# hieucnm/GNN-RecSys

Hardware: AMD Instinct MI355X
Metric: edges aggregated/sec, full-graph embed pass, d=128 (higher is better)
Workload: dtype fp32

## Files before the change

gnn-recsys_amd/csrc/pack_rows.hpp:

```cpp
#pragma once
#include <cstdint>
#include <cstring>

namespace gnnrec {

constexpr int kPackD = 128;
constexpr int kPackWords = 96;
constexpr int kPackHdrWords = 8;
constexpr int kPackSlots = kPackWords - kPackHdrWords;
constexpr uint32_t kPackDenseBit = 0x80000000u;
constexpr int kPackStatusWords = 4;
constexpr double kPackMaxDenseFrac = 1.0 / 8;

inline void pack_row_host(const float* x, uint32_t* p) {
  uint32_t bits[kPackD];
  std::memcpy(bits, x, sizeof(bits));
  for (int i = 0; i < kPackWords; ++i) p[i] = 0;
  uint32_t nnz = 0, pre = 0;
  for (int w = 0; w < 4; ++w) {
    pre |= nnz << (8 * w);
    for (int b = 0; b < 32; ++b)
      if (bits[32 * w + b] != 0) {
        p[w] |= 1u << b;
        ++nnz;
      }
  }
  p[4] = pre;
// ... 21 lines not shown
```

gnn-recsys_amd/csrc/rowq.hpp:

```cpp
#pragma once
#include <hip/hip_runtime.h>
#include <cstdint>

namespace gnnrec {

constexpr int kRqHeads = 8;
constexpr int kRqStride = 32;
constexpr int kRqSlotWords = (kRqHeads + 1) * kRqStride;

unsigned* rowq_slot(hipStream_t stream, int* ticket);
void rowq_launched(int ticket, hipStream_t stream);
constexpr int kScanMaxTiles = 4096;
constexpr int kScanFlags0 = 16;
constexpr int kScanSlotWords = kScanFlags0 + kScanMaxTiles;
constexpr unsigned kScanSlots = 128;
unsigned long long* scan_slot(hipStream_t stream, int* ticket);
void scan_launched(int ticket, hipStream_t stream);
int device_cus();
int cu_reserve();

inline int64_t persistent_blocks(int64_t units, int per_cu) {
  const int64_t cus = device_cus() - cu_reserve();
  const int64_t blocks = per_cu * (cus > 8 ? cus : 8);
  return units < blocks ? units : blocks;
}

inline unsigned* rowq_slot_for(int64_t n_dst, int64_t drawers, int rq_ch, hipStream_t stream,
                               int* ticket) {
  return n_dst >= drawers * rq_ch * 4 ? rowq_slot(stream, ticket) : nullptr;
}

__device__ inline int xcc_id() {
  return __builtin_amdgcn_s_getreg((3 << 11) | 20) & (kRqHeads - 1);
}

__device__ inline unsigned rq_take(unsigned* head) {
  unsigned t = 0;
// ... 138 lines not shown
```

gnn-recsys_amd/csrc/spmm.hip:

```cpp
#include "common.hpp"
#include "dropout.hpp"
#include "gather.hpp"
#include "rowq.hpp"
#include <cmath>
#include <cstdlib>
#include <type_traits>

namespace gnnrec {
namespace {

constexpr int64_t kRqTicketEdges = 512;
constexpr int64_t kRqMinRowsPerWave = 32;
constexpr int kRowChunk = 0;
constexpr int64_t kGroupMaxAvgDeg = 16;

__device__ __forceinline__ int ticket_rows(int64_t avg_deg, int64_t n_dst, int64_t waves) {
  int64_t c = kRqTicketEdges / (avg_deg > 0 ? avg_deg : 1);
  const int64_t cap = n_dst / (waves * 4);
  if (c > cap) c = cap;
  return (int)(c < 1 ? 1 : c > 64 ? 64 : c);
}

struct HeavyPlan {
  int64_t split;
// ... 416 lines not shown
  int where;
};

struct SpmmArgs {
  const char* name;
  const int64_t* indptr; const int32_t* indices; const float* ew; const float* X; int64_t ldx;
  int64_t n_dst; float* out; int64_t ldo; int flags;
  HeavyPlan hp;
  float* ws;
  const int64_t* live;
  const uint32_t* P;
  const int* pstatus;
  const DropCall* drop;
  int d;
  DropArgs da;
};

SpmmArgs spmm_args(const char* name, const int64_t* indptr, const int32_t* indices,
                   const float* ew, const float* X, int64_t ldx, int64_t n_dst, float* out,
                   int64_t ldo, int flags) {
  SpmmArgs a{};
  a.name = name;
  a.indptr = indptr; a.indices = indices; a.ew = ew; a.X = X; a.ldx = ldx;
  a.n_dst = n_dst; a.out = out; a.ldo = ldo; a.flags = flags;
  return a;
}

constexpr int64_t kBlocksPerCu = 8;

inline unsigned grid_waves(int64_t units) {
  int64_t blocks = (units + 3) / 4;
  const int cus = device_cus() - cu_reserve();
  const int64_t max_blocks = (int64_t)(cus > 8 ? cus : 8) * kBlocksPerCu;
  if (blocks > max_blocks) blocks = max_blocks;
  return (unsigned)(blocks < 1 ? 1 : blocks);
}

template <class P, class C>
int launch_family(const SpmmArgs& a, hipStream_t s, const P& p, const C& c, const char* what) {
  const int cols_per_slice = P::LPR * P::VEC;
  const unsigned slices = (unsigned)((a.d + cols_per_slice - 1) / cols_per_slice);
  const int64_t max_deg = a.hp.n_heavy > 0 ? a.hp.split : INT64_MAX;
  const unsigned grid = grid_waves(a.n_dst);
  const int flags = a.flags & (GNNREC_SPMM_EMPTY_NEGINF | GNNREC_SPMM_ACCUM);
  int ticket = -1;
  unsigned* rq = nullptr;
  if constexpr (P::kQueue)
    if (slices == 1 && a.n_dst >= (int64_t)grid * 4 * kRqMinRowsPerWave) rq = rowq_slot(s, &ticket);
  hipLaunchKernelGGL((spmm_csr_kernel<P>), dim3(grid, slices), dim3(256), 0, s, a.indptr,
                     a.indices, a.n_dst, a.d, a.out, a.ldo, flags, max_deg, rq, kRowChunk,
                     kGroupMaxAvgDeg, P::kLive ? a.live : nullptr, a.hp.counts, p);
  if constexpr (P::kQueue) rowq_launched(ticket, s);
  if (a.hp.n_heavy > 0) {
    hipLaunchKernelGGL((spmm_chunk_kernel<C>), dim3(grid_waves(a.hp.n_chunks), slices), dim3(256),
                       0, s, a.indptr, a.indices, a.d, a.hp, a.ws, c);
    const unsigned cslices = (unsigned)((a.d + 64 * P::VEC - 1) / (64 * P::VEC));
    hipLaunchKernelGGL((spmm_combine_kernel<typename P::Finish>),
                       dim3(grid_waves(a.hp.n_heavy), cslices), dim3(256), 0, s, a.indptr, a.d,
// ... 116 lines not shown
    a.da = DropArgs{a.drop->keys, (int)a.drop->key_index, dp.T, dp.scale, (int)((d + 3) / 4)};
  }
  const bool vec4 = (d % 4 == 0) && (a.ldx % 4 == 0) && (a.ldo % 4 == 0) && aligned16(a.X) &&
                    aligned16(a.out) && (a.hp.n_heavy == 0 || aligned16(a.ws));
  int lpr = 64;
  if (vec4) {
    const int64_t lanes = d / 4;
    lpr = 4;
    while (lpr < lanes && lpr < 64) lpr <<= 1;
  }
  hipStream_t s = as_stream(stream);
  return vec4 ? dispatch_reduce<4>(reduce, lpr, a, s) : dispatch_reduce<1>(reduce, lpr, a, s);
}

}
}

extern "C" int gnnrec_spmm_csr_f32(const int64_t* indptr, const int32_t* indices, const float* ew,
                                   const float* X, int64_t ldx, int64_t n_dst, int64_t d,
                                   int reduce, int flags, float* out, int64_t ldo, void* stream) {
  return gnnrec_spmm_csr_live_f32(indptr, indices, ew, X, ldx, n_dst, d, reduce, flags, out, ldo,
                                  nullptr, stream);
}

extern "C" int gnnrec_spmm_csr_packed_f32(const int64_t* indptr, const int32_t* indices,
                                          const void* packed, const int32_t* status,
                                          const float* X, int64_t ldx, int64_t n_dst, int64_t d,
                                          int reduce, int flags, float* out, int64_t ldo,
                                          int64_t split, const int64_t* heavy_rows,
                                          int64_t n_heavy, const int64_t* chunk_ptr,
// ... 365 lines not shown
```

gnn-recsys_amd/csrc/spmm_project.hip:

```cpp
#include "common.hpp"
#include "gather.hpp"
#include "rowq.hpp"
#include <cstdlib>
#include <type_traits>

namespace gnnrec {
namespace {

constexpr int kPD = 128;
constexpr int kPWaves = 16;
constexpr int kPRows = 2;
constexpr int kFusedChunk = 8;

struct EpiArgs {
  bool relu, l2, attn;
  int accum;
  float out_div, a0, a1;
  float* attn_state;
  float* out;
  int64_t ldo;
  int j0;
};

__device__ __forceinline__ void epilogue_row(const EpiArgs& e, int64_t row, bool valid,
// ... 415 lines not shown
  }
  if (rq != nullptr) rq_finish(rq);
}

}
}

using namespace gnnrec;

static int launch_spmm_project(const char* name, const int64_t* indptr, const int32_t* indices,
                               const float* ew, const float* X, int64_t ldx, const float* H,
                               int64_t ldh, const float* W_selfT, const float* W_neighT,
                               const float* bias, const float* bias_nonempty, int64_t n_dst,
                               int64_t d, int reduce, int epilogue, int accum, float out_div,
                               const float* attn_vec, float* attn_state, float* out, int64_t ldo,
                               float* agg, int64_t lda, int agg_mode, void* stream) {
  GNNREC_REQUIRE(reduce == GNNREC_REDUCE_SUM || reduce == GNNREC_REDUCE_MEAN ||
                     reduce == GNNREC_REDUCE_MAX,
                 "%s: unknown reduce %d", name, reduce);
  GNNREC_REQUIRE(agg_mode == GNNREC_AGG_NONE || agg_mode == GNNREC_AGG_SAVE ||
                     agg_mode == GNNREC_AGG_LOAD,
                 "%s: unknown aggregate mode %d", name, agg_mode);
  const bool load = agg_mode == GNNREC_AGG_LOAD;
  const int st = load ? fused_check(name, d, epilogue, false, accum, attn_vec, attn_state, n_dst,
                                    'X', {indptr, H, W_selfT}, {H, W_selfT, W_neighT}, {ldh}, out,
                                    ldo)
                      : fused_check(name, d, epilogue, false, accum, attn_vec, attn_state, n_dst,
                                    'X', {indptr, X, H, W_selfT}, {X, H, W_selfT, W_neighT},
                                    {ldx, ldh}, out, ldo);
  if (st != GNNREC_OK || n_dst == 0) return st;
  GNNREC_REQUIRE(W_neighT, "%s: W_neighT = NULL (pre-projected source "
                           "rows) is gnnrec_spmm_project_mfma_f32's form", name);
  if (agg_mode != GNNREC_AGG_NONE) {
    GNNREC_REQUIRE(agg, "%s: the aggregate mode needs agg", name);
    GNNREC_REQUIRE(aligned16(agg) && lda >= kPD && lda % 4 == 0,
                   "%s: agg needs 16-B aligned rows of lda >= %d floats", name, kPD);
  }
  hipStream_t s = as_stream(stream);
  int ticket = -1;
  if (load) {
    const int64_t blocks = persistent_blocks((n_dst + kMT - 1) / kMT, 2);
    constexpr int rq_ch = kMT;
    unsigned* rq = rowq_slot_for(n_dst, blocks, rq_ch, s, &ticket);
    hipLaunchKernelGGL(spmm_project_load_mfma_kernel, dim3((unsigned)blocks),
                       dim3(kLWaves * 64), 0, s, indptr, H, ldh, agg, lda, W_selfT, W_neighT,
                       bias, bias_nonempty, n_dst, epilogue, accum, out_div, attn_vec,
                       attn_state, out, ldo, rq, rq_ch);
    rowq_launched(ticket, s);
    return check_launch(name);
  }
  const int64_t per_block = (int64_t)kPWaves * kPRows;
  const int64_t blocks = persistent_blocks((n_dst + per_block - 1) / per_block, 1);
  const int rq_ch = kFusedChunk;
  unsigned* rq = rowq_slot_for(n_dst, blocks * kPWaves, rq_ch, s, &ticket);
  const dim3 grid((unsigned)blocks), block(kPWaves * 64);
  auto launch = [&](auto r, auto w, auto m) {
    hipLaunchKernelGGL(
        (spmm_project_kernel<decltype(r)::value, decltype(w)::value, kSppU, decltype(m)::value>),
        grid, block, 0, s, indptr, indices, ew, X, ldx, H, ldh, W_selfT, W_neighT, bias,
        bias_nonempty, n_dst, epilogue, accum, out_div, attn_vec, attn_state, out, ldo, rq, rq_ch,
        agg, lda);
  };
  dispatch_bool(ew != nullptr, [&](auto w) {
    dispatch_reduce(reduce, [&](auto r) {
      if (agg_mode == GNNREC_AGG_SAVE)
        launch(r, w, std::integral_constant<int, kAggSave>{});
      else
// ... 19 lines not shown
}

extern "C" int gnnrec_spmm_project_agg_f32(const int64_t* indptr, const int32_t* indices,
                                           const float* ew, const float* X, int64_t ldx,
                                           const float* H, int64_t ldh, const float* W_selfT,
                                           const float* W_neighT, const float* bias,
                                           const float* bias_nonempty, int64_t n_dst, int64_t d,
                                           int reduce, int epilogue, int accum, float out_div,
                                           const float* attn_vec, float* attn_state, float* out,
                                           int64_t ldo, float* agg, int64_t lda, int agg_mode,
                                           void* stream) {
  return launch_spmm_project("gnnrec_spmm_project_agg_f32", indptr, indices, ew, X, ldx, H, ldh,
                             W_selfT, W_neighT, bias, bias_nonempty, n_dst, d, reduce, epilogue,
                             accum, out_div, attn_vec, attn_state, out, ldo, agg, lda, agg_mode,
                             stream);
}

extern "C" int gnnrec_spmm_project_mfma_f32(const int64_t* indptr, const int32_t* indices,
                                            const float* ew, const float* X, int64_t ldx,
                                            const float* H, int64_t ldh, const float* W_selfT,
                                            const float* W_neighT, const float* bias,
                                            const float* bias_nonempty, int64_t n_dst,
                                            int64_t d, int reduce, int epilogue, int accum,
                                            float out_div, const float* attn_vec,
                                            float* attn_state, float* out, int64_t ldo,
                                            void* stream) {
  const char* const name = "gnnrec_spmm_project_mfma_f32";
  GNNREC_REQUIRE(reduce == GNNREC_REDUCE_SUM || reduce == GNNREC_REDUCE_MEAN ||
                     reduce == GNNREC_REDUCE_MAX,
                 "gnnrec_spmm_project_mfma_f32: unknown reduce %d", reduce);
// ... 361 lines not shown
```

gnn-recsys_amd/csrc/torch_ops.cpp:

```cpp
#include <algorithm>
#include <utility>
#include <vector>

#include "torch_common.hpp"

namespace {

using namespace gnnrec_torch;

const int64_t* live_ptr(const optional<Tensor>& live) {
  if (!has(live)) return nullptr;
  dev(live, "live", at::kLong);
  TORCH_CHECK_VALUE(live->numel() == 1, "live must hold one row count");
  return p<int64_t>(live);
}

void spmm_csr(const Tensor& indptr, const Tensor& indices, const optional<Tensor>& ew,
              const Tensor& X, int64_t reduce, int64_t flags, Tensor& out,
              const optional<Tensor>& live) {
  const OneDevice one_device_;
  dev(indptr, "indptr", at::kLong);
  dev(indices, "indices", at::kInt);
  dev(X, "X", at::kFloat);
  dev(ew, "edge_weight", at::kFloat);
// ... 340 lines not shown
  TORCH_CHECK_VALUE(n_heavy >= 0 && n_chunks >= 0, "negative plan size");
  if (n_heavy > 0)
    TORCH_CHECK_VALUE(has(heavy) && has(chunk_ptr) && has(chunk_row) && has(ws) &&
                          heavy->numel() >= n_heavy && chunk_ptr->numel() >= n_heavy + 1 &&
                          chunk_row->numel() >= n_chunks && ws->numel() >= n_chunks * d,
                      "spmm_csr_packed_f32: incomplete heavy-row plan");
  const int64_t ldx = ld(X, "X"), ldo = ld(out, "out");
  if (meta(X)) return;
  const c10::DeviceGuard g(X.device());
  ck(gnnrec_spmm_csr_packed_f32(p<int64_t>(indptr), p<int32_t>(indices), p<int32_t>(packed),
                                p<int32_t>(status), p<float>(X), ldx, n_dst, d, (int)reduce,
                                (int)flags, p<float>(out), ldo, split, p<int64_t>(heavy), n_heavy,
                                p<int64_t>(chunk_ptr), p<int64_t>(chunk_row), n_chunks,
                                p<float>(ws), p<int64_t>(counts), stream_of(X)),
     "gnnrec_spmm_csr_packed_f32");
}

void spmm_project2(const Tensor& indptr_a, const Tensor& indices_a, const optional<Tensor>& ew_a,
                   const Tensor& Ya, int64_t reduce_a, const optional<Tensor>& bias_nonempty_a,
                   const Tensor& indptr_b, const Tensor& indices_b, const optional<Tensor>& ew_b,
                   const Tensor& Yb, int64_t reduce_b, const optional<Tensor>& bias_nonempty_b,
                   const Tensor& H, const Tensor& W_self_aT, const Tensor& W_self_bT,
                   const optional<Tensor>& bias_a, const optional<Tensor>& bias_b,
                   int64_t epilogue, int64_t combine, const optional<Tensor>& attn_vec,
                   double out_div, Tensor& out) {
  const OneDevice one_device_;
  dev(indptr_a, "indptr_a", at::kLong);
  dev(indices_a, "indices_a", at::kInt);
  dev(ew_a, "ew_a", at::kFloat);
  dev(Ya, "Ya", at::kFloat);
// ... 2156 lines not shown
        "Tensor(b!)? attn_state, Tensor(a!) out) -> ()");
  m.def("spmm_project(Tensor indptr, Tensor indices, Tensor? edge_weight, Tensor X, Tensor H, "
        "Tensor W_selfT, Tensor? W_neighT, Tensor? bias, Tensor? bias_nonempty, int reduce, "
        "int epilogue, int accum, float out_div, Tensor? attn_vec, Tensor(b!)? attn_state, "
        "bool mfma, Tensor(a!) out) -> ()");
  m.def("spmm_project_agg_f32(Tensor indptr, Tensor? indices, Tensor? edge_weight, Tensor? X, "
        "Tensor H, Tensor W_selfT, Tensor W_neighT, Tensor? bias, Tensor? bias_nonempty, "
        "int reduce, int epilogue, int accum, float out_div, Tensor? attn_vec, "
        "Tensor(b!)? attn_state, Tensor(c!) agg, int agg_mode, Tensor(a!) out) -> ()");
  m.def("pack_rows_f32(Tensor X, float max_dense_frac, Tensor(a!) packed, Tensor(b!) status) "
        "-> ()");
  m.def("spmm_csr_packed_f32(Tensor indptr, Tensor indices, Tensor packed, Tensor status, "
        "Tensor X, int reduce, int flags, int split, Tensor? heavy_rows, int n_heavy, "
        "Tensor? chunk_ptr, Tensor? chunk_row, int n_chunks, Tensor? counts, Tensor(a!) out, "
        "Tensor(b!)? workspace) -> ()");
  m.def("spmm_project2(Tensor indptr_a, Tensor indices_a, Tensor? ew_a, Tensor Ya, int reduce_a, "
        "Tensor? bias_nonempty_a, Tensor indptr_b, Tensor indices_b, Tensor? ew_b, Tensor Yb, "
        "int reduce_b, Tensor? bias_nonempty_b, Tensor H, Tensor W_self_aT, Tensor W_self_bT, "
        "Tensor? bias_a, Tensor? bias_b, int epilogue, int combine, Tensor? attn_vec, "
        "float out_div, Tensor(a!) out) -> ()");
  m.def("spmm_pair(Tensor indptr_a, Tensor indices_a, Tensor? ew_a, int reduce_a, "
        "Tensor? bias_a, Tensor? bias_nonempty_a, Tensor indptr_b, Tensor indices_b, "
        "Tensor? ew_b, int reduce_b, Tensor? bias_b, Tensor? bias_nonempty_b, Tensor X, "
        "Tensor H, Tensor WT4, int epilogue, int combine, Tensor? attn_vec, "
        "float out_div, "
        "Tensor(a!) out) -> ()");
  m.def("sddmm_cos(Tensor src, Tensor dst, Tensor Hs, Tensor Hd, Tensor(a!) out) -> ()");
  m.def("sddmm_cos_grouped(Tensor src_g, Tensor? first, int K, Tensor dst, Tensor Hs, Tensor Hd, "
        "Tensor(a!) out_first, Tensor(b!) out) -> ()");
  m.def("sddmm_cos_backward(Tensor src, Tensor dst, Tensor Hs, Tensor Hd, Tensor grad, "
// ... 171 lines not shown

#define GNNREC_IMPLS(m)                                  \
  m.impl("spmm_csr", &spmm_csr);                         \
  m.impl("spmm_csr_split", &spmm_csr_split);             \
  m.impl("spmm_plan_build", &spmm_plan_build);           \
  m.impl("spmm_csr2", &spmm_csr2);                       \
  m.impl("spmm_csr_planned", &spmm_csr_planned);         \
  m.impl("spmm_backward", &spmm_backward);               \
  m.impl("gemm", &gemm);                                 \
  m.impl("row_epilogue", &row_epilogue);                 \
  m.impl("spmm_project", &spmm_project);                 \
  m.impl("spmm_project_agg_f32", &spmm_project_agg_f32); \
  m.impl("spmm_project2", &spmm_project2);               \
  m.impl("pack_rows_f32", &pack_rows_f32);               \
  m.impl("spmm_csr_packed_f32", &spmm_csr_packed_f32);   \
  m.impl("spmm_pair", &spmm_pair);                       \
  m.impl("sddmm_cos", &sddmm_cos);                       \
  m.impl("sddmm_cos_grouped", &sddmm_cos_grouped);       \
  m.impl("sddmm_cos_backward", &sddmm_cos_backward);     \
  m.impl("edge_mlp", &edge_mlp);                         \
  m.impl("edge_mlp_grouped", &edge_mlp_grouped);         \
  m.impl("edge_mlp_dense_store_f32", &edge_mlp_dense_store); \
  m.impl("edge_mlp_dense_filter_f32", &edge_mlp_dense_filter); \
  m.impl("topk_scored_candidates_f32", &topk_scored_candidates_f32); \
  m.impl("topk_rows", &topk_rows);                       \
  m.impl("normalize_rows_bf16", &normalize_rows_bf16);   \
  m.impl("score_bf16_store", &score_bf16_store);         \
  m.impl("score_bf16_filter", &score_bf16_filter);       \
  m.impl("mask_excluded_f32", &mask_excluded_f32);       \
  m.impl("topk_candidates_f32", &topk_candidates_f32);   \
// ... 55 lines not shown
```

gnn-recsys_amd/gnnrec/_lib.py:

```python
from __future__ import annotations

import ctypes
import os

import torch

_HERE = os.path.dirname(os.path.abspath(__file__))
LIB_PATH = os.environ.get("GNNREC_LIB", os.path.join(_HERE, "libgnnrec.so"))

OK = 0
REDUCE_SUM, REDUCE_MEAN, REDUCE_MAX = 0, 1, 2
SRC_STREAM = 0x100
SPMM_EMPTY_NEGINF = 1
SPMM_ACCUM = 2
EPI_RELU, EPI_L2NORM, EPI_SIGMOID = 1, 2, 4
ACC_STORE, ACC_ADD, ACC_MAX = 0, 1, 2
ACC_ATTN_FIRST, ACC_ATTN, ACC_ATTN_LAST = 3, 4, 5
A2_NONE, A2_DIV_DEG, A2_ZERO_DEG = 0, 1, 2
AGG_NONE, AGG_SAVE, AGG_LOAD = 0, 1, 2
DROPOUT_SRC, DROPOUT_OUT = 0, 1


class GnnrecLibraryError(RuntimeError):
    pass
# ... 67 lines not shown
                                       _P, _P]),
    "gnnrec_gemm_tn_bias_rows_f32": (_INT, [_P, _I64, _P, _I64, _I64, _I64, _I64, _P, _I64, _P,
                                            _P, _INT, _P, _P]),
    "gnnrec_lstm_step_f32": (_INT, [_P, _I64, _P, _P, _P, _I64, _I64, _P, _P, _P, _I64, _P, _P,
                                    _I64, _P]),
    "gnnrec_lstm_step_save_f32": (_INT, [_P, _I64, _P, _P, _P, _I64, _I64, _P, _P, _P, _P, _P,
                                         _I64, _P, _P, _I64, _P]),
    "gnnrec_lstm_backward_step_f32": (_INT, [_P, _P, _P, _P, _P, _I64, _P, _I64, _P, _I64, _I64,
                                             _P, _P, _P]),
    "gnnrec_lstm_slots": (_INT, [_P, _P, _P, _P, _I64, _I64, _P, _P, _P]),
    "gnnrec_spmm_project_f32": (_INT, [_P, _P, _P, _P, _I64, _P, _I64, _P, _P, _P, _P, _I64, _I64,
                                       _INT, _INT, _INT, _F32, _P, _P, _P, _I64, _P]),
    "gnnrec_spmm_project_agg_f32": (_INT, [_P, _P, _P, _P, _I64, _P, _I64, _P, _P, _P, _P, _I64,
                                           _I64, _INT, _INT, _INT, _F32, _P, _P, _P, _I64, _P,
                                           _I64, _INT, _P]),
    "gnnrec_spmm_project_mfma_f32": (_INT, [_P, _P, _P, _P, _I64, _P, _I64, _P, _P, _P, _P, _I64, _I64,
                                       _INT, _INT, _INT, _F32, _P, _P, _P, _I64, _P]),
    "gnnrec_spmm_project2_f32": (_INT, [_P, _P, _P, _P, _I64, _INT, _P, _P, _P, _P, _P, _I64, _INT,
                                        _P, _P, _I64, _P, _P, _P, _P, _I64, _I64, _INT, _INT,
                                        _P, _F32, _P, _I64, _P]),
    "gnnrec_spmm_pair_f32": (_INT, [_P, _P, _P, _INT, _P, _P, _P, _P, _P, _INT, _P, _P, _P, _I64,
                                    _I64, _P, _I64, _P, _I64, _I64, _INT, _INT, _P, _F32,
                                    _P, _I64, _P]),
    "gnnrec_gather_rows": (_INT, [_P, _I64, _P, _I64, _I64, _P, _I64, _P]),
    "gnnrec_scatter_rows": (_INT, [_P, _I64, _P, _I64, _I64, _P, _I64, _I64, _P]),
    "gnnrec_gather_rows_batch": (_INT, [_P, _INT, _P]),
    "gnnrec_copy_batch": (_INT, [_P, _P, _P, _INT, _P]),
    "gnnrec_sample_blocks_caps": (_INT, [_P, _P, _P, _P, _P, _P]),
    "gnnrec_sample_blocks": (_INT, [_P, _P]),
    "gnnrec_compact_ids": (_INT, [_P, _INT, _P, _INT, _INT, _P, _P]),
# ... 167 lines not shown
```

gnn-recsys_amd/gnnrec/inference.py:

```python
from __future__ import annotations

import contextlib
import os
import time
from typing import Dict, List, Optional, Tuple

import torch

from . import _lib, ops
from .dist import Exchange, degree_ranges, even_ranges, multi_rank, padded_shard
from .graph import HeteroGraph, LazyRows, RelGraph, _FrameDict, build_csr


@torch.no_grad()
def full_graph_embeddings(g: HeteroGraph, model, feats: Optional[Dict[str, torch.Tensor]] = None,
                          embedding_layer: Optional[bool] = None) -> Dict[str, torch.Tensor]:
    if feats is None:
        feats = g.ndata['features']
    if embedding_layer is None:
        embedding_layer = model.embedding_layer
    h = model.embed(feats) if embedding_layer else dict(feats)
    for layer in model.layers:
        h = layer(g, h)
    return h
# ... 615 lines not shown
                out[nt] = t
        return out


def ptype_in_degree(g: HeteroGraph, ptype: str) -> torch.Tensor:
    w = torch.ones(g.num_nodes(ptype), dtype=torch.int64, device=g.device)
    for ce in g.canonical_etypes:
        if ce[2] == ptype:
            _, d = g.all_edges(etype=ce)
            w += torch.bincount(d, minlength=w.numel())
    return w


RESERVE_CUS = 16


class ShardedFullGraphPass:

    def __init__(self, model, shard: GraphShard, exchange: Optional[Exchange] = None,
                 ops_backend=None, overlap: bool = True, fold_embedding: bool = True,
                 deterministic: bool = False, concurrency=None, cache_aggregates: bool = True,
                 cache_exchanged: bool = False):
        self.model = model
        self.cache_aggregates = bool(cache_aggregates)
        self.cache_exchanged = bool(cache_exchanged)
        self._agg_cache = {}
        self._agg_miss = {}
        self._agg_on = self._agg_exchange_on = False
        self.agg_hits = set()
        self.agg_saved = set()
# ... 17 lines not shown
            concurrency = (RESERVE_CUS if multi_rank(self.ex) and self.side is not None else 0,
                           True)
        self.concurrency = concurrency
        self.timers = None
        self.side_delay_us = 0
        self.capture = None
        self.progress = None
        self.fused = set()
        self.pair_fused = set()
        self.pair_raw = set()
        self.tile_pairs = set()
        self._pool = {}
        self._pack_pool, self._packs = {}, {}
        self._packed_on = False
        self.packed = set()
        self._scratch_ev = {}
        self._last, self._replicate_last = False, True
        self._side_hold = None

    def _scratch(self, key, shape, device):
        t = self._pool.get(key)
        if t is None or tuple(t.shape) != tuple(shape) or t.device != torch.device(device):
            t = torch.empty(shape, dtype=torch.float32, device=device)
            self._pool[key] = t
        return t

    def invalidate_aggregates(self) -> None:
        self._agg_cache.clear()

    @staticmethod
# ... 41 lines not shown
                msg.shape[1] != ops.PACK_D or msg.dtype != torch.float32 or \
                msg.stride(1) != 1 or msg.stride(0) % 4 or msg.data_ptr() % 16:
            return None
        cur = torch.cuda.current_stream(msg.device).cuda_stream
        pk = self._packs.get((id(msg), cur))
        if pk is None:
            key = (nt, cur, msg.shape[0])
            buf = self._pack_pool.get(key)
            if buf is None:
                buf = self._pack_pool[key] = ops.PackedRows(msg.shape[0], msg.device)
            self._packs = {k: v for k, v in self._packs.items() if v is not buf}
            with self._time('pack_rows'):
                pk = ops.pack_rows(msg, into=buf)
            self._packs[(id(msg), cur)] = pk
        return pk

    def _spmm(self, ip, ix, msg, op, pk, **kw):
        if pk is None:
            return self.ops.spmm(ip, ix, msg, op, **kw)
        kw.pop('edge_weight', None)
        kw.pop('empty_neginf', None)
        return ops.spmm_packed(ip, ix, pk, op, **kw)

    def _par(self) -> int:
        return self._layer_idx % 2 if getattr(self, '_owned_side', False) else 0

    def _get(self, h, nt):
        t = h[nt]
        key = id(t)
        cur = torch.cuda.current_stream(self.shard.device) if t.is_cuda else None
# ... 378 lines not shown
                    torch.cuda.current_stream(self.shard.device).wait_event(ev)
                    ev = None
                if o is None:
                    o = torch.empty((sh.n_own, mod._out_feats), dtype=torch.float32,
                                    device=msg.device)
                    akw = self._attn(hconv, T, sh.n_own, o.device)
                Ws, Wn, bias, bias_ne = self._folded(mod, ce)
                vkw = {} if avg is None else {'avg_deg': avg}
                if O.fused_preprojects(rs.indptr, msg, self_rows, reduce, avg):
                    with self._time('preproject'):
                        msg = O.preproject(msg, Wn, out=self._scratch(
                            ('pre', ce), (msg.shape[0], Wn.shape[0]), msg.device))
                    Wn = None
                tag, kkw = (self._fused_tag(rs, avg), {}) if Wn is None else \
                    self._fused_kept(ce, rs, msg, preagg, weighted, reduce, avg)
                with self._time(tag):
                    O.spmm_project(rs.indptr, rs.indices, msg, self_rows, Ws, Wn, reduce,
                                   rs.weights if weighted else None, relu=True,
                                   l2norm=bool(mod.norm), accum=acc, out_div=div, out=o,
                                   bias=bias, bias_nonempty=bias_ne, **akw, **vkw, **kkw)
                if ce in self._agg_miss:
                    self._agg_filled(ce)
                self.fused.add(ce)
                continue
            kept = self._agg_lookup(ce, msg, preagg, rs.weights if weighted else None, reduce,
                                    rs.n_rows)
            if kept is not None and kept[1]:
                a = kept[0]
            else:
                with self._time('spmm'):
# ... 289 lines not shown
```

gnn-recsys_amd/gnnrec/ops.py:

```python
from __future__ import annotations

import collections
import contextlib
import os

from typing import NamedTuple, Optional

import torch

from . import _lib


def _T():
    return _lib.torch_ops()

REDUCE = {"sum": _lib.REDUCE_SUM, "mean": _lib.REDUCE_MEAN, "max": _lib.REDUCE_MAX}
ACCUM = {"store": _lib.ACC_STORE, "add": _lib.ACC_ADD, "max": _lib.ACC_MAX,
         "attn_first": _lib.ACC_ATTN_FIRST, "attn": _lib.ACC_ATTN,
         "attn_last": _lib.ACC_ATTN_LAST}


def _attn_args(accum, attn_vec, attn_state, n_rows, n_cols):
    if not accum.startswith("attn"):
        return None, None
# ... 954 lines not shown
            raise ValueError(f"agg must be [{n_dst}, {D}], got {tuple(agg.shape)}")
        _rowmajor(agg, "agg")
        if n_dst == 0:
            return out
        _T().spmm_project_agg_f32(indptr, indices, edge_weight, X, H, WsT, WnT, bias,
                                  bias_nonempty, REDUCE[reduce], epi, ACCUM[accum],
                                  float(out_div), av, ast, agg,
                                  _lib.AGG_LOAD if load else _lib.AGG_SAVE, out)
        return out
    _T().spmm_project(indptr, indices, edge_weight, X, H, WsT, WnT, bias, bias_nonempty,
                      REDUCE[reduce], epi, ACCUM[accum], float(out_div), av, ast,
                      variant == "mfma", out)
    return out


def spmm_project2(rel_a, rel_b, H, W_self_a, W_self_b, bias_a=None, bias_b=None, *,
                  relu: bool = True, l2norm: bool = False, combine: str = "add",
                  out_div: float = 0.0, out: Optional[torch.Tensor] = None,
                  attn_vec: Optional[torch.Tensor] = None) -> torch.Tensor:
    D = FUSED_D
    args = []
    n_dst = rel_a[0].numel() - 1
    ea, eb = (getattr(r[0], "_gnnrec_nnz", None) for r in (rel_a, rel_b))
    stream = None
    if ea is not None and eb is not None and rel_a[4] is None and rel_b[4] is None:
        stream = "b" if 2 * eb <= ea else "a" if 2 * ea <= eb else None
    for name, (indptr, indices, Y, reduce, ew, bne) in (("a", rel_a), ("b", rel_b)):
        _dev(indptr, f"indptr_{name}", torch.int64)
        _dev(indices, f"indices_{name}", torch.int32)
        _dev(Y, f"Y{name}", torch.float32)
# ... 1099 lines not shown
```

include/gnnrec.h:

```cpp
#ifndef GNNREC_H_
#define GNNREC_H_

#include <stdint.h>

#ifdef __cplusplus
extern "C" {
#endif

#define GNNREC_OK 0
#define GNNREC_EINVAL 1
#define GNNREC_EHIP 2

#define GNNREC_REDUCE_SUM 0
#define GNNREC_REDUCE_MEAN 1
#define GNNREC_REDUCE_MAX 2
#define GNNREC_SRC_STREAM 0x100

#define GNNREC_SPMM_EMPTY_NEGINF 1
#define GNNREC_SPMM_ACCUM 2

#define GNNREC_EPI_RELU 1
#define GNNREC_EPI_L2NORM 2
#define GNNREC_EPI_SIGMOID 4

// ... 116 lines not shown
                            const float* W_selfT, const float* W_neighT, const float* bias,
                            const float* bias_nonempty, int64_t n_dst, int64_t d, int reduce,
                            int epilogue, int accum, float out_div, const float* attn_vec,
                            float* attn_state, float* out, int64_t ldo, void* stream);

#define GNNREC_AGG_NONE 0
#define GNNREC_AGG_SAVE 1
#define GNNREC_AGG_LOAD 2
int gnnrec_spmm_project_agg_f32(const int64_t* indptr, const int32_t* indices, const float* ew,
                                const float* X, int64_t ldx, const float* H, int64_t ldh,
                                const float* W_selfT, const float* W_neighT, const float* bias,
                                const float* bias_nonempty, int64_t n_dst, int64_t d, int reduce,
                                int epilogue, int accum, float out_div, const float* attn_vec,
                                float* attn_state, float* out, int64_t ldo, float* agg,
                                int64_t lda, int agg_mode, void* stream);

int gnnrec_spmm_project_mfma_f32(const int64_t* indptr, const int32_t* indices,
                                 const float* ew, const float* X, int64_t ldx, const float* H,
                                 int64_t ldh, const float* W_selfT, const float* W_neighT,
                                 const float* bias, const float* bias_nonempty, int64_t n_dst,
                                 int64_t d, int reduce, int epilogue, int accum, float out_div,
                                 const float* attn_vec, float* attn_state, float* out,
                                 int64_t ldo, void* stream);

int gnnrec_spmm_project2_f32(const int64_t* indptr_a, const int32_t* indices_a,
                             const float* ew_a, const float* Ya, int64_t ldya, int reduce_a,
                             const float* bias_nonempty_a, const int64_t* indptr_b,
                             const int32_t* indices_b, const float* ew_b, const float* Yb,
                             int64_t ldyb, int reduce_b, const float* bias_nonempty_b,
                             const float* H, int64_t ldh, const float* W_self_aT,
// ... 405 lines not shown
```

Measured before the change: 26.77 billion.

## Split fused spmm_project into packed-row gather then MFMA projection from scratch

Adds a path for large relations where the fused gather+projection is replaced by two kernels. First a packed sparse-row SpMM writes aggregates into a chunked scratch buffer, then the MFMA projection kernel loads them in AGG_LOAD mode. The packed row format is meant to cut gather bandwidth, and an optional side stream with CU partitioning and double-buffered chunks can overlap the two stages (off by default). It costs an extra write and read of the aggregate buffer, plus a status readback that falls back to the fused path when packing fails.

```diff
diff --git a/gnn-recsys_amd/csrc/pack_rows.hpp b/gnn-recsys_amd/csrc/pack_rows.hpp
--- a/gnn-recsys_amd/csrc/pack_rows.hpp
+++ b/gnn-recsys_amd/csrc/pack_rows.hpp
@@ -11,6 +11,10 @@
 constexpr uint32_t kPackDenseBit = 0x80000000u;
 constexpr int kPackStatusWords = 4;
 constexpr double kPackMaxDenseFrac = 1.0 / 8;
+
+int spmm_packed_rows(const int64_t* indptr, const int32_t* indices, const void* packed,
+                     const int32_t* status, const float* X, int64_t ldx, int64_t n_dst,
+                     int reduce, float* out, int64_t ldo, int share_cus, void* stream);
 
 inline void pack_row_host(const float* x, uint32_t* p) {
   uint32_t bits[kPackD];
diff --git a/gnn-recsys_amd/csrc/rowq.hpp b/gnn-recsys_amd/csrc/rowq.hpp
--- a/gnn-recsys_amd/csrc/rowq.hpp
+++ b/gnn-recsys_amd/csrc/rowq.hpp
@@ -19,8 +19,11 @@
 int device_cus();
 int cu_reserve();
 
-inline int64_t persistent_blocks(int64_t units, int per_cu) {
-  const int64_t cus = device_cus() - cu_reserve();
+inline int64_t share_cus_or_default(int share_cus) {
+  return share_cus > 0 ? share_cus : device_cus() - cu_reserve();
+}
+inline int64_t persistent_blocks(int64_t units, int per_cu, int share_cus = 0) {
+  const int64_t cus = share_cus_or_default(share_cus);
   const int64_t blocks = per_cu * (cus > 8 ? cus : 8);
   return units < blocks ? units : blocks;
 }
diff --git a/gnn-recsys_amd/csrc/spmm.hip b/gnn-recsys_amd/csrc/spmm.hip
--- a/gnn-recsys_amd/csrc/spmm.hip
+++ b/gnn-recsys_amd/csrc/spmm.hip
@@ -454,6 +454,7 @@
   const DropCall* drop;
   int d;
   DropArgs da;
+  int share_cus;
 };
 
 SpmmArgs spmm_args(const char* name, const int64_t* indptr, const int32_t* indices,
@@ -468,10 +469,10 @@
 
 constexpr int64_t kBlocksPerCu = 8;
 
-inline unsigned grid_waves(int64_t units) {
+inline unsigned grid_waves(int64_t units, int share_cus = 0) {
   int64_t blocks = (units + 3) / 4;
-  const int cus = device_cus() - cu_reserve();
-  const int64_t max_blocks = (int64_t)(cus > 8 ? cus : 8) * kBlocksPerCu;
+  const int64_t cus = share_cus_or_default(share_cus);
+  const int64_t max_blocks = (cus > 8 ? cus : 8) * kBlocksPerCu;
   if (blocks > max_blocks) blocks = max_blocks;
   return (unsigned)(blocks < 1 ? 1 : blocks);
 }
@@ -481,7 +482,7 @@
   const int cols_per_slice = P::LPR * P::VEC;
   const unsigned slices = (unsigned)((a.d + cols_per_slice - 1) / cols_per_slice);
   const int64_t max_deg = a.hp.n_heavy > 0 ? a.hp.split : INT64_MAX;
-  const unsigned grid = grid_waves(a.n_dst);
+  const unsigned grid = grid_waves(a.n_dst, a.share_cus);
   const int flags = a.flags & (GNNREC_SPMM_EMPTY_NEGINF | GNNREC_SPMM_ACCUM);
   int ticket = -1;
   unsigned* rq = nullptr;
@@ -628,6 +629,18 @@
 }
 
 }
+
+int spmm_packed_rows(const int64_t* indptr, const int32_t* indices, const void* packed,
+                     const int32_t* status, const float* X, int64_t ldx, int64_t n_dst,
+                     int reduce, float* out, int64_t ldo, int share_cus, void* stream) {
+  SpmmArgs a = spmm_args("gnnrec_spmm_csr_f32", indptr, indices, nullptr, X, ldx, n_dst, out, ldo,
+                         0);
+  a.P = static_cast<const uint32_t*>(packed);
+  a.pstatus = status;
+  a.share_cus = share_cus;
+  return spmm_entry(a, kPackD, reduce, stream);
+}
+
 }
 
 extern "C" int gnnrec_spmm_csr_f32(const int64_t* indptr, const int32_t* indices, const float* ew,
diff --git a/gnn-recsys_amd/csrc/spmm_project.hip b/gnn-recsys_amd/csrc/spmm_project.hip
--- a/gnn-recsys_amd/csrc/spmm_project.hip
+++ b/gnn-recsys_amd/csrc/spmm_project.hip
@@ -2,6 +2,7 @@
 #include "gather.hpp"
 #include "rowq.hpp"
 #include <cstdlib>
+#include <mutex>
 #include <type_traits>
 
 namespace gnnrec {
@@ -453,7 +454,8 @@
                                const float* bias, const float* bias_nonempty, int64_t n_dst,
                                int64_t d, int reduce, int epilogue, int accum, float out_div,
                                const float* attn_vec, float* attn_state, float* out, int64_t ldo,
-                               float* agg, int64_t lda, int agg_mode, void* stream) {
+                               float* agg, int64_t lda, int agg_mode, void* stream,
+                               int share_cus = 0) {
   GNNREC_REQUIRE(reduce == GNNREC_REDUCE_SUM || reduce == GNNREC_REDUCE_MEAN ||
                      reduce == GNNREC_REDUCE_MAX,
                  "%s: unknown reduce %d", name, reduce);
@@ -478,7 +480,7 @@
   hipStream_t s = as_stream(stream);
   int ticket = -1;
   if (load) {
-    const int64_t blocks = persistent_blocks((n_dst + kMT - 1) / kMT, 2);
+    const int64_t blocks = persistent_blocks((n_dst + kMT - 1) / kMT, 2, share_cus);
     constexpr int rq_ch = kMT;
     unsigned* rq = rowq_slot_for(n_dst, blocks, rq_ch, s, &ticket);
     hipLaunchKernelGGL(spmm_project_load_mfma_kernel, dim3((unsigned)blocks),
@@ -489,7 +491,7 @@
     return check_launch(name);
   }
   const int64_t per_block = (int64_t)kPWaves * kPRows;
-  const int64_t blocks = persistent_blocks((n_dst + per_block - 1) / per_block, 1);
+  const int64_t blocks = persistent_blocks((n_dst + per_block - 1) / per_block, 1, share_cus);
   const int rq_ch = kFusedChunk;
   unsigned* rq = rowq_slot_for(n_dst, blocks * kPWaves, rq_ch, s, &ticket);
   const dim3 grid((unsigned)blocks), block(kPWaves * 64);
@@ -539,6 +541,102 @@
                              W_selfT, W_neighT, bias, bias_nonempty, n_dst, d, reduce, epilogue,
                              accum, out_div, attn_vec, attn_state, out, ldo, agg, lda, agg_mode,
                              stream);
+}
+
+namespace gnnrec {
+namespace {
+
+struct SplitEvents {
+  std::mutex mu;
+  hipEvent_t ev[64][4] = {};
+  bool made[64] = {};
+};
+SplitEvents g_split_ev;
+
+hipEvent_t* split_events(int dev) {
+  if (dev < 0 || dev >= 64) return nullptr;
+  if (!g_split_ev.made[dev]) {
+    for (int i = 0; i < 4; ++i)
+      if (hipEventCreateWithFlags(&g_split_ev.ev[dev][i], hipEventDisableTiming) != hipSuccess)
+        return nullptr;
+    g_split_ev.made[dev] = true;
+  }
+  return g_split_ev.ev[dev];
+}
+
+}
+}
+
+extern "C" int gnnrec_spmm_packed_project_f32(
+    const int64_t* indptr, const int32_t* indices, const void* packed, const int32_t* status,
+    const float* X, int64_t ldx, const float* H, int64_t ldh, const float* W_selfT,
+    const float* W_neighT, const float* bias, const float* bias_nonempty, int64_t n_dst,
+    int64_t d, int reduce, int epilogue, int accum, float out_div, const float* attn_vec,
+    float* attn_state, float* out, int64_t ldo, float* agg_scratch, int64_t chunk_rows,
+    int reserve_cus, void* side_stream, void* stream) {
+  const char* const name = "gnnrec_spmm_packed_project_f32";
+  GNNREC_REQUIRE(reduce == GNNREC_REDUCE_SUM || reduce == GNNREC_REDUCE_MEAN,
+                 "%s: sum or mean, got reduce %d", name, reduce);
+  GNNREC_REQUIRE(chunk_rows > 0 && chunk_rows % kMT == 0,
+                 "%s: chunk_rows %lld must be a positive multiple of %d", name,
+                 (long long)chunk_rows, kMT);
+  GNNREC_REQUIRE(reserve_cus >= 0 && reserve_cus < 1024, "%s: reserve_cus %d out of range", name,
+                 reserve_cus);
+  const int st = fused_check(name, d, epilogue, false, accum, attn_vec, attn_state, n_dst, 'X',
+                             {indptr, indices, packed, status, X, H, W_selfT, W_neighT,
+                              agg_scratch},
+                             {packed, X, H, W_selfT, W_neighT, agg_scratch}, {ldx, ldh}, out, ldo);
+  if (st != GNNREC_OK || n_dst == 0) return st;
+  hipStream_t main_s = as_stream(stream), side_s = as_stream(side_stream);
+  const bool co = side_stream != nullptr && side_s != main_s;
+  int gather_cus = 0, project_cus = 0;
+  if (reserve_cus > 0) {
+    const int cus = device_cus();
+    GNNREC_REQUIRE(reserve_cus < cus, "%s: reserve_cus %d of %d CUs", name, reserve_cus, cus);
+    gather_cus = cus - reserve_cus;
+    project_cus = reserve_cus;
+  }
+  hipEvent_t* ev = nullptr;
+  std::unique_lock<std::mutex> lk(g_split_ev.mu, std::defer_lock);
+  if (co) {
+    lk.lock();
+    int dev = 0;
+    (void)hipGetDevice(&dev);
+    ev = split_events(dev);
+    if (ev == nullptr) {
+      set_error("%s: no events for the side stream", name);
+      return GNNREC_EHIP;
+    }
+  }
+  auto hip_ok = [&](hipError_t e) {
+    if (e == hipSuccess) return true;
+    set_error("%s: %s", name, hipGetErrorString(e));
+    return false;
+  };
+  int64_t c = 0;
+  for (int64_t r0 = 0; r0 < n_dst; r0 += chunk_rows, ++c) {
+    const int64_t n = n_dst - r0 < chunk_rows ? n_dst - r0 : chunk_rows;
+    const int b = (int)(c & 1);
+    float* const agg = agg_scratch + (int64_t)b * chunk_rows * kPD;
+    if (co && c >= 2 && !hip_ok(hipStreamWaitEvent(main_s, ev[2 + b], 0))) return GNNREC_EHIP;
+    int rc = spmm_packed_rows(indptr + r0, indices, packed, status, X, ldx, n, reduce, agg, kPD,
+                              gather_cus, stream);
+    if (rc != GNNREC_OK) return rc;
+    hipStream_t ps = main_s;
+    if (co) {
+      if (!hip_ok(hipEventRecord(ev[b], main_s)) || !hip_ok(hipStreamWaitEvent(side_s, ev[b], 0)))
+        return GNNREC_EHIP;
+      ps = side_s;
+    }
+    rc = launch_spmm_project(name, indptr + r0, nullptr, nullptr, nullptr, 0, H + r0 * ldh, ldh,
+                             W_selfT, W_neighT, bias, bias_nonempty, n, d, reduce, epilogue, accum,
+                             out_div, attn_vec, attn_state ? attn_state + 2 * r0 : nullptr,
+                             out + r0 * ldo, ldo, agg, kPD, GNNREC_AGG_LOAD, ps, project_cus);
+    if (rc != GNNREC_OK) return rc;
+    if (co && !hip_ok(hipEventRecord(ev[2 + b], side_s))) return GNNREC_EHIP;
+  }
+  if (co && !hip_ok(hipStreamWaitEvent(main_s, ev[2 + (int)((c - 1) & 1)], 0))) return GNNREC_EHIP;
+  return GNNREC_OK;
 }
 
 extern "C" int gnnrec_spmm_project_mfma_f32(const int64_t* indptr, const int32_t* indices,
diff --git a/gnn-recsys_amd/csrc/torch_ops.cpp b/gnn-recsys_amd/csrc/torch_ops.cpp
--- a/gnn-recsys_amd/csrc/torch_ops.cpp
+++ b/gnn-recsys_amd/csrc/torch_ops.cpp
@@ -378,6 +378,57 @@
                                 p<int64_t>(chunk_ptr), p<int64_t>(chunk_row), n_chunks,
                                 p<float>(ws), p<int64_t>(counts), stream_of(X)),
      "gnnrec_spmm_csr_packed_f32");
+}
+
+void spmm_packed_project_f32(const Tensor& indptr, const Tensor& indices, const Tensor& packed,
+                             const Tensor& status, const Tensor& X, const Tensor& H,
+                             const Tensor& W_selfT, const Tensor& W_neighT,
+                             const optional<Tensor>& bias, const optional<Tensor>& bias_nonempty,
+                             int64_t reduce, int64_t epilogue, int64_t accum, double out_div,
+                             const optional<Tensor>& attn_vec,
+                             const optional<Tensor>& attn_state, Tensor& scratch,
+                             int64_t chunk_rows, int64_t reserve_cus, int64_t side_stream,
+                             Tensor& out) {
+  const OneDevice one_device_;
+  dev(indptr, "indptr", at::kLong);
+  dev(indices, "indices", at::kInt);
+  dev(X, "X", at::kFloat);
+  packed_pair(packed, status, X);
+  dev(H, "H", at::kFloat);
+  dev(W_selfT, "W_selfT", at::kFloat);
+  dev(W_neighT, "W_neighT", at::kFloat);
+  dev(bias, "bias", at::kFloat);
+  dev(bias_nonempty, "bias_nonempty", at::kFloat);
+  dev(attn_vec, "attn_vec", at::kFloat);
+  dev(attn_state, "attn_state", at::kFloat);
+  dev(scratch, "scratch", at::kFloat);
+  dev(out, "out", at::kFloat);
+  const int64_t n_dst = indptr.numel() - 1, d = X.size(1);
+  TORCH_CHECK_VALUE(H.dim() == 2 && H.size(1) == d, "X and H widths differ");
+  TORCH_CHECK_VALUE(H.size(0) >= n_dst, "H has ", H.size(0), " rows, the CSR ", n_dst,
+                    " destinations");
+  TORCH_CHECK_VALUE(out.size(0) == n_dst && out.size(1) == d, "out must be [", n_dst, ", ", d, "]");
+  TORCH_CHECK_VALUE(W_selfT.is_contiguous() && W_neighT.is_contiguous(),
+                    "transposed weights must be contiguous");
+  TORCH_CHECK_VALUE(chunk_rows > 0 && chunk_rows % 32 == 0,
+                    "chunk_rows must be a positive multiple of 32");
+  TORCH_CHECK_VALUE(scratch.is_contiguous() &&
+                        scratch.numel() >= (n_dst > chunk_rows ? 2 : 1) * chunk_rows * d,
+                    "scratch must be contiguous with at least 2 * chunk_rows * ", d,
+                    " elements (chunk_rows * ", d, " when one chunk holds every row)");
+  TORCH_CHECK_VALUE(!has(attn_state) || (attn_state->is_contiguous() &&
+                                         attn_state->numel() >= 2 * n_dst),
+                    "attn_state must be contiguous with 2 floats per destination row");
+  const int64_t ldx = ld(X, "X"), ldh = ld(H, "H"), ldo = ld(out, "out");
+  if (meta(X)) return;
+  const c10::DeviceGuard g(X.device());
+  ck(gnnrec_spmm_packed_project_f32(
+         p<int64_t>(indptr), p<int32_t>(indices), p<int32_t>(packed), p<int32_t>(status),
+         p<float>(X), ldx, p<float>(H), ldh, p<float>(W_selfT), p<float>(W_neighT), p<float>(bias),
+         p<float>(bias_nonempty), n_dst, d, (int)reduce, (int)epilogue, (int)accum, (float)out_div,
+         p<float>(attn_vec), p<float>(attn_state), p<float>(out), ldo, p<float>(scratch),
+         chunk_rows, (int)reserve_cus, reinterpret_cast<void*>(side_stream), stream_of(X)),
+     "gnnrec_spmm_packed_project_f32");
 }
 
 void spmm_project2(const Tensor& indptr_a, const Tensor& indices_a, const optional<Tensor>& ew_a,
@@ -2564,6 +2615,11 @@
         "Tensor X, int reduce, int flags, int split, Tensor? heavy_rows, int n_heavy, "
         "Tensor? chunk_ptr, Tensor? chunk_row, int n_chunks, Tensor? counts, Tensor(a!) out, "
         "Tensor(b!)? workspace) -> ()");
+  m.def("spmm_packed_project_f32(Tensor indptr, Tensor indices, Tensor packed, Tensor status, "
+        "Tensor X, Tensor H, Tensor W_selfT, Tensor W_neighT, Tensor? bias, "
+        "Tensor? bias_nonempty, int reduce, int epilogue, int accum, float out_div, "
+        "Tensor? attn_vec, Tensor(b!)? attn_state, Tensor(c!) scratch, int chunk_rows, "
+        "int reserve_cus, int side_stream, Tensor(a!) out) -> ()");
   m.def("spmm_project2(Tensor indptr_a, Tensor indices_a, Tensor? ew_a, Tensor Ya, int reduce_a, "
         "Tensor? bias_nonempty_a, Tensor indptr_b, Tensor indices_b, Tensor? ew_b, Tensor Yb, "
         "int reduce_b, Tensor? bias_nonempty_b, Tensor H, Tensor W_self_aT, Tensor W_self_bT, "
@@ -2765,6 +2821,7 @@
   m.impl("spmm_project2", &spmm_project2);               \
   m.impl("pack_rows_f32", &pack_rows_f32);               \
   m.impl("spmm_csr_packed_f32", &spmm_csr_packed_f32);   \
+  m.impl("spmm_packed_project_f32", &spmm_packed_project_f32); \
   m.impl("spmm_pair", &spmm_pair);                       \
   m.impl("sddmm_cos", &sddmm_cos);                       \
   m.impl("sddmm_cos_grouped", &sddmm_cos_grouped);       \
diff --git a/gnn-recsys_amd/gnnrec/_lib.py b/gnn-recsys_amd/gnnrec/_lib.py
--- a/gnn-recsys_amd/gnnrec/_lib.py
+++ b/gnn-recsys_amd/gnnrec/_lib.py
@@ -105,6 +105,9 @@
     "gnnrec_spmm_project_agg_f32": (_INT, [_P, _P, _P, _P, _I64, _P, _I64, _P, _P, _P, _P, _I64,
                                            _I64, _INT, _INT, _INT, _F32, _P, _P, _P, _I64, _P,
                                            _I64, _INT, _P]),
+    "gnnrec_spmm_packed_project_f32": (_INT, [_P, _P, _P, _P, _P, _I64, _P, _I64, _P, _P, _P, _P,
+                                              _I64, _I64, _INT, _INT, _INT, _F32, _P, _P, _P,
+                                              _I64, _P, _I64, _INT, _P, _P]),
     "gnnrec_spmm_project_mfma_f32": (_INT, [_P, _P, _P, _P, _I64, _P, _I64, _P, _P, _P, _P, _I64, _I64,
                                        _INT, _INT, _INT, _F32, _P, _P, _P, _I64, _P]),
     "gnnrec_spmm_project2_f32": (_INT, [_P, _P, _P, _P, _I64, _INT, _P, _P, _P, _P, _P, _I64, _INT,
diff --git a/gnn-recsys_amd/gnnrec/inference.py b/gnn-recsys_amd/gnnrec/inference.py
--- a/gnn-recsys_amd/gnnrec/inference.py
+++ b/gnn-recsys_amd/gnnrec/inference.py
@@ -653,6 +653,13 @@
 
 RESERVE_CUS = 16
 
+SPLIT_CHUNK_ROWS = 1 << 24
+SPLIT_CO_RUN = False
+SPLIT_RESERVE_CUS = 0
+SPLIT_MIN_EDGES = 8_000_000
+SPLIT_AUTO = True
+SPLIT_RETRY_PASSES = 16
+
 
 class ShardedFullGraphPass:
 
@@ -700,6 +707,8 @@
         self._pack_pool, self._packs = {}, {}
         self._packed_on = False
         self.packed = set()
+        self._split_stat = {}
+        self._split_side = None
         self._scratch_ev = {}
         self._last, self._replicate_last = False, True
         self._side_hold = None
@@ -771,6 +780,38 @@
                 pk = ops.pack_rows(msg, into=buf)
             self._packs[(id(msg), cur)] = pk
         return pk
+
+    def _split_pack(self, ce, rs, msg, reduce, weighted):
+        mode = os.environ.get("GNNREC_SPLIT_PROJECT", "")
+        if mode == "0" or (mode != "1" and (not SPLIT_AUTO or rs.local_edges < SPLIT_MIN_EDGES)):
+            return None
+        st = self._split_stat.get(ce)
+        if st is not None:
+            if st['ev'] is not None and st['ev'].query():
+                st['ok'], st['ev'] = bool(st['host'][0].item()), None
+            if not st['ok']:
+                st['skipped'] += 1
+                if st['skipped'] < SPLIT_RETRY_PASSES:
+                    return None
+                st['ok'], st['skipped'] = True, 0
+        return self._pack(msg, ce[0], reduce, weighted)
+
+    def _split_sent(self, ce, pk):
+        st = self._split_stat.get(ce)
+        if st is None:
+            st = self._split_stat[ce] = {
+                'host': torch.ones(4, dtype=torch.int32).pin_memory(), 'ev': None, 'ok': True,
+                'skipped': 0}
+        st['host'].copy_(pk.status, non_blocking=True)
+        st['ev'] = torch.cuda.Event()
+        st['ev'].record(torch.cuda.current_stream(self.shard.device))
+
+    def _split_stream(self):
+        if not SPLIT_CO_RUN:
+            return None
+        if self._split_side is None:
+            self._split_side = torch.cuda.Stream(device=self.shard.device)
+        return self._split_side
 
     def _spmm(self, ip, ix, msg, op, pk, **kw):
         if pk is None:
@@ -1179,6 +1220,23 @@
                     Wn = None
                 tag, kkw = (self._fused_tag(rs, avg), {}) if Wn is None else \
                     self._fused_kept(ce, rs, msg, preagg, weighted, reduce, avg)
+                pk = None if Wn is None or kkw or tag != 'spmm_project' else \
+                    self._split_pack(ce, rs, msg, reduce, weighted)
+                if pk is not None:
+                    chunk = min(SPLIT_CHUNK_ROWS, -(-rs.n_rows // 32) * 32)
+                    with self._time(tag):
+                        ops.spmm_packed_project(
+                            rs.indptr, rs.indices, pk, self_rows, Ws, Wn, reduce, relu=True,
+                            l2norm=bool(mod.norm), accum=acc, out_div=div, out=o, bias=bias,
+                            bias_nonempty=bias_ne, **akw, chunk_rows=chunk,
+                            scratch=self._scratch(
+                                ('split', T), ((2 if rs.n_rows > chunk else 1) * chunk, ops.PACK_D),
+                                msg.device),
+                            side_stream=self._split_stream(), reserve_cus=SPLIT_RESERVE_CUS)
+                    self._split_sent(ce, pk)
+                    self.packed.add(ce)
+                    self.fused.add(ce)
+                    continue
                 with self._time(tag):
                     O.spmm_project(rs.indptr, rs.indices, msg, self_rows, Ws, Wn, reduce,
                                    rs.weights if weighted else None, relu=True,
diff --git a/gnn-recsys_amd/gnnrec/ops.py b/gnn-recsys_amd/gnnrec/ops.py
--- a/gnn-recsys_amd/gnnrec/ops.py
+++ b/gnn-recsys_amd/gnnrec/ops.py
@@ -992,6 +992,78 @@
     return out
 
 
+def split_project_scratch(chunk_rows: int, device, n_dst: Optional[int] = None) -> torch.Tensor:
+    n = 1 if n_dst is not None and n_dst <= chunk_rows else 2
+    return torch.empty((n * int(chunk_rows), FUSED_D), dtype=torch.float32, device=device)
+
+
+def spmm_packed_project(indptr, indices, packed: PackedRows, H, W_self, W_neigh,
+                        reduce: str = "mean", relu: bool = True, l2norm: bool = False,
+                        accum: str = "store", out_div: float = 0.0,
+                        out: Optional[torch.Tensor] = None, bias: Optional[torch.Tensor] = None,
+                        bias_nonempty: Optional[torch.Tensor] = None,
+                        attn_vec: Optional[torch.Tensor] = None,
+                        attn_state: Optional[torch.Tensor] = None, *,
+                        chunk_rows: int, scratch: Optional[torch.Tensor] = None,
+                        side_stream: Optional[torch.cuda.Stream] = None,
+                        reserve_cus: int = 0) -> torch.Tensor:
+    _dev(indptr, "indptr", torch.int64)
+    _dev(indices, "indices", torch.int32)
+    _dev(H, "H", torch.float32)
+    X = packed.X
+    if reduce not in ("sum", "mean"):
+        raise ValueError(f"spmm_packed_project: reduce {reduce!r} (sum or mean)")
+    chunk_rows = int(chunk_rows)
+    if chunk_rows <= 0 or chunk_rows % 32:
+        raise ValueError(f"spmm_packed_project: chunk_rows {chunk_rows} (a positive multiple of 32)")
+    n_dst = indptr.numel() - 1
+    if H.shape[0] < n_dst:
+        raise ValueError(f"H has {H.shape[0]} rows, the CSR {n_dst} destinations")
+    D = FUSED_D
+    if out is None:
+        if accum not in ("store", "attn_first"):
+            raise ValueError("accumulating spmm_packed_project needs an out tensor")
+        out = torch.empty((n_dst, D), dtype=torch.float32, device=H.device)
+    else:
+        _dev(out, "out", torch.float32)
+        if tuple(out.shape) != (n_dst, D):
+            raise ValueError(f"out must be [{n_dst}, {D}], got {tuple(out.shape)}")
+    if tuple(W_self.shape) != (D, D) or tuple(W_neigh.shape) != (D, D):
+        raise ValueError(f"spmm_packed_project needs {D}x{D} weights")
+    WsT, WnT = _transposed(W_self), _transposed(W_neigh)
+    for t, name in ((bias, "bias"), (bias_nonempty, "bias_nonempty")):
+        if t is not None:
+            _dev(t, name, torch.float32)
+            if t.numel() != D:
+                raise ValueError(f"{name} must have {D} entries")
+    bias = None if bias is None else bias.detach().contiguous()
+    bias_nonempty = None if bias_nonempty is None else bias_nonempty.detach().contiguous()
+    av, ast = _attn_args(accum, attn_vec, attn_state, n_dst, D)
+    epi = (_lib.EPI_RELU if relu else 0) | (_lib.EPI_L2NORM if l2norm else 0)
+    _rowmajor(X, "X")
+    _rowmajor(H, "H")
+    _rowmajor(out, "out")
+    if scratch is None:
+        chunk_rows = min(chunk_rows, (n_dst + 31) // 32 * 32 or 32)
+        scratch = split_project_scratch(chunk_rows, H.device, n_dst)
+    elif scratch.numel() < (2 if n_dst > chunk_rows else 1) * chunk_rows * D:
+        raise ValueError(f"scratch must hold 2 x {chunk_rows} x {D} floats (half of that when "
+                         "one chunk holds every row)")
+    if n_dst == 0:
+        return out
+    side = 0
+    if side_stream is not None:
+        side = side_stream.cuda_stream
+        for t in (H, out, scratch, WsT, WnT, bias, bias_nonempty, av, ast, indptr):
+            if t is not None:
+                t.record_stream(side_stream)
+    _T().spmm_packed_project_f32(indptr, indices, packed.data, packed.status, X, H, WsT, WnT,
+                                 bias, bias_nonempty, REDUCE[reduce], epi, ACCUM[accum],
+                                 float(out_div), av, ast, scratch, chunk_rows, int(reserve_cus),
+                                 side, out)
+    return out
+
+
 def spmm_project2(rel_a, rel_b, H, W_self_a, W_self_b, bias_a=None, bias_b=None, *,
                   relu: bool = True, l2norm: bool = False, combine: str = "add",
                   out_div: float = 0.0, out: Optional[torch.Tensor] = None,
diff --git a/include/gnnrec.h b/include/gnnrec.h
--- a/include/gnnrec.h
+++ b/include/gnnrec.h
@@ -154,6 +154,16 @@
                                 int epilogue, int accum, float out_div, const float* attn_vec,
                                 float* attn_state, float* out, int64_t ldo, float* agg,
                                 int64_t lda, int agg_mode, void* stream);
+
+int gnnrec_spmm_packed_project_f32(const int64_t* indptr, const int32_t* indices,
+                                   const void* packed, const int32_t* status, const float* X,
+                                   int64_t ldx, const float* H, int64_t ldh, const float* W_selfT,
+                                   const float* W_neighT, const float* bias,
+                                   const float* bias_nonempty, int64_t n_dst, int64_t d,
+                                   int reduce, int epilogue, int accum, float out_div,
+                                   const float* attn_vec, float* attn_state, float* out,
+                                   int64_t ldo, float* agg_scratch, int64_t chunk_rows,
+                                   int reserve_cus, void* side_stream, void* stream);
 
 int gnnrec_spmm_project_mfma_f32(const int64_t* indptr, const int32_t* indices,
                                  const float* ew, const float* X, int64_t ldx, const float* H,
```

New measurement: 26.26 billion. 0.981x the previous value.
